# LikeLy-Journey/SegmenTron

Measured on AMD Instinct MI355X. Metric: images/sec fwd+bwd DeepLabv3+_xception65 @1025x2049, higher is better.
Workload: dtype bf16; 1 GPU; DeepLabv3+_xception65 train step (fwd + CE loss + bwd + SGD) @1025x2049, batch 2/GPU (BASELINE.json configs[2]); global_batch=2, bn=BN, parallelism=dp1, full_size=True

## Files before the change

include/segmentron_hip.h:

```cpp
#ifndef SEGMENTRON_HIP_H
#define SEGMENTRON_HIP_H
#ifdef __cplusplus
extern "C" {
#endif

const char* seg_last_error(void);
int seg_version(void);

int seg_fast_div_host(const int* s, long n, int d, int* q);
int seg_fast_div_exact(long s, long d);
int seg_fast_div_max_quot(long* out);

int seg_conv_gemm_fwd(int dtype, const void* x, long ldx, int N, int Hi, int Wi, int C,
                      const void* w, int O, int KH, int KW, int stride, int pad, int dil,
                      int pro_mode, const float* pro_scale, const float* pro_shift,
                      const float* bias, void* y, long ldy, int Ho, int Wo, int out_H, int out_W,
                      int out_s, float* stat_partial, const void* ep_x, long ldep,
                      const float* ep_c0, const float* ep_c1, int tconv, void* stream);
int seg_conv_gemm_tiles_m(int N, int Ho, int Wo);

int seg_conv_gemm_wgrad(int dtype, const void* x, long ldx, int N, int Hi, int Wi, int C,
                        const void* dy, long lddy, int Ho, int Wo, int O, int KH, int KW,
                        int stride, int pad, int dil, int pro_mode, const float* pro_scale,
                        const float* pro_shift, float* partial, int splits, void* stream);
// ... 194 lines not shown
                      const float* ta, const void* b, long ldb, const float* sb, const float* tb,
                      const void* res, long ldres, const float* w, int dil, void* ga, long ldga,
                      void* gb, long ldgb, int N, int H, int W, int n, float* pw, float* pa,
                      long pa_pitch, int pa_col, float* pb, int rows, void* stream);
int seg_fpe_bn_bwd_apply(int dtype, const void* g, long ldg, const void* x, long ldx,
                         const float* scale, const float* c0, const float* c1, void* dx, long lddx,
                         long rows, int n, void* stream);
int seg_meu_rows(int N, int h, int w, int C, int high);
int seg_meu_fwd(int dtype, const void* L, long ldl, const float* sl, const float* tl, const void* Hr,
                long ldh, const float* sh, const float* th, const float* a, const float* wsa,
                void* out, long ldo, float* sa, int N, int h, int w, int h2, int w2, int C,
                void* stream);
int seg_meu_bwd_low(int dtype, const void* g, long ldg, const void* L, long ldl, const float* sl,
                    const float* tl, const void* Hr, long ldh, const float* sh, const float* th,
                    const float* a, const float* wsa, const float* sa, void* dL, long lddl, int N,
                    int h, int w, int h2, int w2, int C, float* p_a, float* p_bn, int rows,
                    void* stream);
int seg_meu_bwd_high(int dtype, const void* g, long ldg, const float* sa, const void* Hr, long ldh,
                     const float* dpool, void* dH, long lddh, int N, int h, int w, int h2, int w2,
                     int C, float* p_bn, int rows, void* stream);

int seg_skip_pool_fwd(int dtype, const void* y, long ldy, int N, int H, int W, int C, int pro_mode,
                      const float* pro_scale, const float* pro_shift, void* skip, long ldskip,
                      void* pooled, long ldpool, void* stream);
int seg_skip_pool_bwd_rows(int dtype, int N, int H, int W, int C);
int seg_skip_pool_bwd(int dtype, const void* g_skip, long ldgs, const void* g_pool, long ldgp,
                      const void* y, long ldy, int N, int H, int W, int C, int pro_mode,
                      const float* pro_scale, const float* pro_shift, void* gx, long ldgx,
                      float* partial, int rows, void* stream);
int seg_bilinear_pad_fwd(int dtype, const void* x, long ldx, int N, int Hi, int Wi, int C,
                         int pro_mode, const float* pro_scale, const float* pro_shift, void* y,
                         long ldy, int Ho, int Wo, int Hd, int Wd, int top, int left,
                         int align_corners, void* stream);
int seg_bilinear_pad_bwd(int dtype, void* gx, long ldgx, int N, int Hi, int Wi, int C, const void* gy,
                         long ldgy, int Ho, int Wo, int Hd, int Wd, int top, int left,
                         int align_corners, void* stream);

int seg_bilinear_fwd(int dtype, const void* x, long ldx, int N, int Hi, int Wi, int C,
                     int pro_mode, const float* pro_scale, const float* pro_shift,
                     const float* chan_mul, void* y, long ldy, int Ho, int Wo, int align_corners,
                     void* stream);
int seg_bilinear_bwd(int dtype, void* gx, long ldgx, int N, int Hi, int Wi, int C, const void* gy,
                     long ldgy, int Ho, int Wo, int align_corners, void* stream);
int seg_nearest_add(int dtype, const void* x, long ldx, int mode_x, const float* sx,
                    const float* tx, const void* r, long ldr, int mode_r, const float* sr,
                    const float* tr, int shift, int post_relu, void* y, long ldy, int N, int H,
                    int W, int C, void* stream);
int seg_nearest_sum_bwd(int dtype, const void* g, long ldg, int N, int H, int W, int C, int shift,
                        void* gr, long ldgr, void* stream);
int seg_upsample_to_nchw(int dtype, const void* x, long ldx, int N, int Hi, int Wi, int C,
                         float* out, int Ho, int Wo, int align_corners, void* stream);
int seg_upsample_to_nchw_bwd(int dtype, void* gx, long ldgx, int N, int Hi, int Wi, int C,
                             const float* gy, int Ho, int Wo, int align_corners, void* stream);
int seg_nchw_to_nhwc_pad(int dtype, const float* x, int N, int Cin, int H, int W, void* y,
                         void* stream);

int seg_upsample_ce_blocks(int N, int H, int W);
int seg_upsample_ce_bwd_ws_bytes(int N, int H, int Wi, int C);
int seg_upsample_ce_fwd(int dtype, const void* lo, long ld, int N, int Hi, int Wi, int C,
                        const long* target, int H, int W, long ignore_index, int align_corners,
                        double* ws, float* loss_out, void* stream);
int seg_upsample_ce_bwd(int dtype, const void* lo, long ld, int N, int Hi, int Wi, int C,
                        const long* target, int H, int W, long ignore_index, int align_corners,
                        const float* loss_out, const float* grad_out, void* dlo, long lddlo,
                        float* ws, long ws_bytes, void* stream);

int seg_dup_ce_blocks(int dtype, long ld, int N, int h, int w, int s, int C);
int seg_dup_ce_fwd(int dtype, const void* lo, long ld, int N, int h, int w, int s, int C,
                   const long* target, long ignore_index, double* ws, float* loss_out,
                   void* stream);
int seg_dup_ce_bwd(int dtype, const void* lo, long ld, int N, int h, int w, int s, int C,
                   const long* target, long ignore_index, const float* loss_out,
                   const float* grad_out, void* dlo, long lddlo, void* stream);
int seg_dup_to_nchw(int dtype, const void* lo, long ld, int N, int h, int w, int s, int C,
                    float* out, void* stream);
int seg_dup_to_nchw_bwd(int dtype, void* gx, long ldgx, int N, int h, int w, int s, int C,
                        const float* gy, void* stream);

int seg_point_sample(int dtype_x, const void* x, long sn, long sp, long sc, int N, int H, int W,
                     int C, const float* pts, int P, int nearest, int dtype_y, void* y, long ldy,
                     int col, void* stream);
int seg_point_sample_bwd_ws(int N, int H, int W, int P);
int seg_point_sample_bwd(int dtype_g, const void* g, long ldg, int col, const float* pts, int N,
                         int P, int H, int W, int C, int dtype_x, void* dx, long lddx, int* ws,
                         void* stream);
int seg_point_uncertainty(int dtype, const void* x, long sn, long sp, long sc, int N, int H, int W,
                          int C, const float* pts, int P, float* u, void* stream);
int seg_point_topk_ws(int N, long L);
int seg_point_topk(const float* keys, int N, long L, int K, long* idx, int* ws, void* stream);
int seg_point_coords(const float* over, const long* idx, int N, int L, int K, const float* cover,
                     int P, int H, int W, float* pts, void* stream);
int seg_point_scatter(int dtype_r, const void* rend, long ldr, const long* idx, int N, int P,
                      int C, float* y, long sn, long sp, long sc, void* stream);
int seg_point_resize(int dtype, const void* x, long sn, long sp, long sc, int N, int Hi, int Wi,
                     int C, float* y, int Ho, int Wo, int align_corners, void* stream);
int seg_point_ce_blocks(long R);
int seg_point_ce_fwd(int dtype, const void* x, long ldx, long R, int C, const long* target,
                     long ignore_index, double* ws, float* loss_out, void* stream);
int seg_point_ce_bwd(int dtype, const void* x, long ldx, long R, int C, const long* target,
                     long ignore_index, const float* loss_out, const float* grad_out, void* dx,
                     long lddx, void* stream);

int seg_dwconv3x3_s2_grid_y(int C, int N, int H, int W);
int seg_dwconv3x3_s2_bwd_fused(int dtype, const void* dy, long lddy, const void* x, long ldx, int N,
                               int H, int W, int C, const float* w_c9, int pro_mode,
                               const float* pro_scale, const float* pro_shift, void* g, long ldg,
// ... 97 lines not shown
```

segmentron_amd/functional.py:

```python
import contextlib
import dataclasses
import os
import weakref

import torch
import torch.distributed as dist
import torch.nn as nn

from . import hip_ops as K
from . import parallel
from .hip_ops import PRO_AFFINE, PRO_NONE, PRO_RELU


class BNState:
    __slots__ = ("gamma", "beta", "mean", "invstd", "scale", "shift", "count", "training", "group")

    def __init__(self, gamma, beta, mean, invstd, scale, shift, count, training, group=None):
        self.gamma, self.beta = gamma, beta
        self.mean, self.invstd, self.scale, self.shift = mean, invstd, scale, shift
        self.count, self.training, self.group = count, training, group


RELU, RELU6 = 1, 5


class Act:
    __slots__ = ("t", "bn", "relu", "park")

    def __init__(self, t, bn=None, relu=False, park=None):
        self.t, self.bn, self.relu = t, bn, relu
        self.park = park

    @property
    def pro(self):
        mode = (PRO_AFFINE if self.bn is not None else PRO_NONE) | int(self.relu)
        if self.bn is None:
            return (mode, None, None)
        return (mode, self.bn.scale, self.bn.shift)

    @property
    def params(self):
        if self.bn is None:
            return None, None
        return self.bn.gamma, self.bn.beta

    def with_relu(self):
        return Act(self.t, self.bn, self.relu or True)

    @property
    def shape(self):
        return self.t.shape


_sync_group = parallel.sync_group


class GradFork:
    __slots__ = ("g", "kind", "closed", "coef")
    POST, PRE, RAW, SUM = 0, 1, 2, 3

    def __init__(self, kind=0):
        self.g, self.kind, self.closed, self.coef = None, kind, False, None

    def take(self):
        g, self.g = self.g, None
        return g

    def can_park(self, kind, g, like):
        return (self.kind == kind and self.g is None and not self.closed
                and g.dtype == like.dtype and tuple(g.shape) == tuple(like.shape))


def uses_batch_stats(bn):
    return not getattr(bn, "frozen", False) and (bn.training or bn.running_mean is None)


def finish_bn(bn, partial, count, mean_offset=None, y=None):
    use_batch = uses_batch_stats(bn)
    if not use_batch:
        scale, shift = eval_affine(bn)
        invstd = mean = None
        if torch.is_grad_enabled():
            mean = bn.running_mean
            invstd = torch.rsqrt(bn.running_var + bn.eps)
        return BNState(bn.weight, bn.bias, mean, invstd, scale, shift, count, False)
    if count <= 1 and _sync_group(bn) is None:
        raise ValueError("Expected more than 1 value per channel when training, got count=%d"
                         % count)
    group = _sync_group(bn)
    cnt = float(count)
    momentum = bn.momentum if bn.momentum is not None else 0.1
    track = bn.training and getattr(bn, "track_running_stats", False) \
        and bn.running_mean is not None
    rm, rv = (bn.running_mean, bn.running_var) if track else (None, None)
    if track:
        note_running_stats_changed()
    if group is None and y is not None and count <= K.SMALL_BN_ROWS:
        mean, invstd, scale, shift = K.bn_finalize_small(y, bn.weight, bn.bias, bn.eps, momentum,
                                                         rm, rv, mean_offset)
    elif group is None:
        mean, invstd, scale, shift = K.bn_finalize_p(partial, cnt, bn.weight, bn.bias, bn.eps,
                                                     momentum, rm, rv, mean_offset)
    else:
        C = partial.shape[-1]
        naive = parallel.is_naive_sync(bn)
        if naive:
            rm = rv = None
        box = parallel.mailbox(group)
        small = y is not None and count * dist.get_world_size(group) <= K.SMALL_BN_ROWS
        if box is not None and small:
            mean, invstd, scale, shift, cnt = K.bn_finalize_small_sync(
                box, y, bn.weight, bn.bias, bn.eps, momentum, rm, rv, mean_offset)
# ... 430 lines not shown
        else:
            dy_full = dy
        Cx = x.shape[-1]
        Ow = dy_full.shape[-1]
        dWp = K.conv_wgrad(x, dy_full, Ow, KH, KW, s.stride, s.pad, s.dil, s.pro)[:O]
        G = s.groups
        if G > 1:
            dW = block_diag_grad(dWp.view(O, Cx), G)
        elif KH == 1 and KW == 1 and Cx == Cw:
            dW = dWp.view(O, Cw, 1, 1)
        else:
            dW = dWp.view(O, KH, KW, Cx)[..., :Cw].permute(0, 3, 1, 2).contiguous()
        dbias = None
        if ctx.has_bias and s.drop_bias:
            dbias = torch.zeros(O, dtype=torch.float32, device=dy.device)
        elif ctx.has_bias:
            dbias = K.bn_bwd_reduce(dy_full, dy_full, (PRO_NONE, None, None))[:O].float()
        dx = dgamma = dbeta = None
        if ctx.needs_input_grad[0]:
            Op, dt = dy_full.shape[-1], x.dtype

            def rows(w2d):
                return w2d if Cx == Cw else torch.nn.functional.pad(w2d, (0, 0, 0, Cx - Cw))
            if G > 1:
                wt = cached_pack(weight, ("dgrad_bd", G, Op, dt), lambda: pack_conv_weight_dgrad(
                    block_diag_weight(weight, G), Op, dt))
            elif KH == 1 and KW == 1 and Op == O and Cx == Cw and weight.dtype == torch.float32:
                wt = packed_pointwise(weight, True, dt)
            else:
                wt = cached_pack(weight, ("dgrad", Op, dt, Cx),
                                 lambda: rows(pack_conv_weight_dgrad(weight, Op, dt)))
            res = None
            if s.fork is not None and s.fork.g is not None:
                res = s.fork.take()
            inplace = res is not None and getattr(s.fork, "inplace", False) \
                and tuple(res.shape) == tuple(x.shape) and _sum_n_operand_ok(res, K.vec_of(dt))
            if s.stride == 1 and res is not None and KH == 1 and KW == 1 and s.bn_in is None \
                    and not s.relu and (Cx == Cw or inplace) and Cx % K.vec_of(dt) == 0 \
                    and res.dtype == dt:
                g, _ = K.conv_gemm(dy_full, wt, Cx, 1, 1, 1, 0, 1, out=res if inplace else None,
                                   ep=(res, _const(Cx, x.device, 0.0), _const(Cx, x.device, -1.0)))
                res = None
            elif s.stride == 1:
                g, _ = K.conv_gemm(dy_full, wt, Cx, KH, KW, 1, s.dil * (KH - 1) - s.pad, s.dil)
            elif KH == 1 and KW == 1 and s.pad == 0:
                g, _ = K.conv_gemm(dy_full, wt, Cx, 1, 1, 1, 0, 1,
                                   scatter=(x.shape[1], x.shape[2], s.stride))
            else:
                wt = cached_pack(weight, ("tconv", Op, dt, Cx),
                                 lambda: rows(pack_conv_weight_tconv(weight, Op, dt)))
                g, _ = K.conv_gemm(dy_full, wt, Cx, KH, KW, s.stride, s.pad, s.dil,
                                   tconv_out_hw=(x.shape[1], x.shape[2]))
            p = s.park
            if res is None and p is not None and p.kind in (GradFork.SUM, GradFork.PRE) \
                    and p.can_park(p.kind, g, x):
                if p.kind == GradFork.PRE:
                    bn = s.bn_in
                    mode = PRO_AFFINE | int(s.relu)
                    partial = K.bn_bwd_reduce_partial(g, x, (mode, bn.scale, bn.shift))
                    dgamma, dbeta, c0, c1, _ = _bn_bwd_finish(partial, bn)
                    p.coef = (mode, c0, c1)
                p.g = g
                return None, dgamma, dbeta, dW, dbias, None
            dx, dgamma, dbeta = bn_input_backward(g, x, s.bn_in, s.relu, inplace=True)
            if res is not None:
                dx = dx + res
        elif s.fork is not None:
            s.fork.g = None
        return dx, dgamma, dbeta, dW, dbias, None


_ONES = {}


def _const(c, device, value):
    key = (c, str(device), float(value))
    if key not in _ONES:
        _ONES[key] = torch.full((c,), float(value), dtype=torch.float32, device=device)
    return _ONES[key]


def _ones(c, device):
    return _const(c, device, 1.0)


class _FoldConvFn(torch.autograd.Function):

    @staticmethod
    def forward(ctx, x, in_gamma, in_beta, weight, spec):
        O, C = weight.shape[0], weight.shape[1]
        bn = spec.bn_in
        w2d = weight.detach().view(O, C)
        wp, wpt, bp = K.fold_weights(w2d, bn.scale, bn.shift, x.dtype,
                                     want_transpose=ctx.needs_input_grad[0])
        spec.mean_offset = bp
        bias = None if spec.drop_const else bp
        y, spec.partial = K.conv_gemm(x, wp, O, 1, 1, spec.stride, 0, 1, None, bias, spec.out,
                                      spec.want_stats)
        spec.out = None
        ctx.spec = spec
        ctx.wpt = wpt
        ctx.save_for_backward(x, weight)
        return y

    @staticmethod
    def backward(ctx, dy):
        x, weight = ctx.saved_tensors
        s = ctx.spec
        bn = s.bn_in
        O, C = weight.shape[0], weight.shape[1]
        if K.nhwc(dy)[4] % K.vec_of(dy.dtype) != 0:
            dy = dy.contiguous()
        dwp = K.conv_wgrad(x, dy, O, 1, 1, s.stride, 0, 1, None, raw_partial=True)
        db = None
        if not s.drop_const:
            db = K.bn_bwd_reduce(dy, dy, (PRO_NONE, None, None))[:O].float()
        dW, dsdt = K.fold_bwd_reduce(weight.detach().view(O, C), dwp, bn.scale, bn.shift, db)
        if _bn_sums_exchanged_in_kernel(bn):
            dgamma, dbeta, c0, c1 = K.fold_bwd_finalize_sync(
                parallel.mailbox(bn.group), dsdt, bn.count, bn.mean, bn.invstd, bn.gamma, bn.scale,
                parallel.grad_scale(bn.group))
        else:
# ... 1910 lines not shown
```

segmentron_amd/hip_ops.py:

```python
import torch

from ._lib import LIB

PRO_NONE, PRO_RELU, PRO_AFFINE, PRO_AFFINE_RELU = 0, 1, 2, 3
_DT = {torch.float32: 0, torch.bfloat16: 1}


def vec_of(dtype):
    return 8 if dtype == torch.bfloat16 else 4


_raw_stream = getattr(torch._C, "_cuda_getCurrentRawStream", None)


def _stream():
    if _raw_stream is not None:
        return _raw_stream(torch.cuda.current_device())
    return torch.cuda.current_stream().cuda_stream


def _p(t):
    return 0 if t is None else t.data_ptr()


# ... 958 lines not shown
    return torch.tensor([[float(a * b) for b in ws] for a in hs], device=device)


def bilinear(x, out_hw, pro=None, chan_mul=None, align_corners=True, out=None):
    N, Hi, Wi, C, ldx = nhwc(x)
    Ho, Wo = out_hw
    mode, s, t = _pro(pro)
    if out is None:
        out = torch.empty((N, Ho, Wo, C), dtype=x.dtype, device=x.device)
    ldy = nhwc(out)[4]
    LIB.call("seg_bilinear_fwd", _DT[x.dtype], _p(x), ldx, N, Hi, Wi, C, mode, _p(s), _p(t),
             _p(chan_mul), _p(out), ldy, Ho, Wo, int(align_corners), _stream())
    return out


def bilinear_bwd(gy, in_hw, align_corners=True):
    N, Ho, Wo, C, ldgy = nhwc(gy)
    Hi, Wi = in_hw
    gx = torch.empty((N, Hi, Wi, C), dtype=gy.dtype, device=gy.device)
    LIB.call("seg_bilinear_bwd", _DT[gy.dtype], _p(gx), C, N, Hi, Wi, C, _p(gy), ldgy, Ho, Wo,
             int(align_corners), _stream())
    return gx


def upsample_to_nchw(x, C, out_hw, align_corners=True):
    N, Hi, Wi, _, ldx = nhwc(x)
    Ho, Wo = out_hw
    out = torch.empty((N, C, Ho, Wo), dtype=torch.float32, device=x.device)
    LIB.call("seg_upsample_to_nchw", _DT[x.dtype], _p(x), ldx, N, Hi, Wi, C, _p(out), Ho, Wo,
             int(align_corners), _stream())
    return out


def upsample_to_nchw_bwd(gy, in_hw, dtype, pitch, align_corners=True):
    if not gy.is_cuda or gy.dtype != torch.float32:
        raise RuntimeError("upsample_to_nchw_bwd needs a float32 HIP device tensor")
    N, C, Ho, Wo = gy.shape
    Hi, Wi = in_hw
    gy = gy.contiguous()
    gx = torch.empty((N, Hi, Wi, pitch), dtype=dtype, device=gy.device)
    LIB.call("seg_upsample_to_nchw_bwd", _DT[dtype], _p(gx), pitch, N, Hi, Wi, C, _p(gy), Ho, Wo,
             int(align_corners), _stream())
    return gx


def nchw_to_nhwc_pad(x, dtype):
    if not x.is_cuda:
        raise RuntimeError("segmentron_amd ops need HIP device tensors (no CPU fallback)")
    N, Cin, H, W = x.shape
    x = x.contiguous().float()
    y = torch.empty((N, H, W, vec_of(dtype)), dtype=dtype, device=x.device)
    LIB.call("seg_nchw_to_nhwc_pad", _DT[dtype], _p(x), N, Cin, H, W, _p(y), _stream())
    return y


def upsample_ce_fwd(lo, target, out_hw, ignore_index, align_corners=True):
    N, Hi, Wi, C, ld = nhwc(lo)
    H, W = out_hw
    if not target.is_cuda or target.dtype != torch.int64 or tuple(target.shape) != (N, H, W):
        raise RuntimeError("upsample_ce: target must be an int64 HIP tensor [N, H, W] = %s, got %s"
                           % ((N, H, W), tuple(target.shape)))
    target = target.contiguous()
    blocks = LIB.query("seg_upsample_ce_blocks", N, H, W)
    ws = torch.empty(2 * blocks, dtype=torch.float64, device=lo.device)
    out = torch.empty(2, dtype=torch.float32, device=lo.device)
    LIB.call("seg_upsample_ce_fwd", _DT[lo.dtype], _p(lo), ld, N, Hi, Wi, C, _p(target), H, W,
             int(ignore_index), int(align_corners), _p(ws), _p(out), _stream())
    return out


def upsample_ce_bwd(lo, target, out_hw, ignore_index, loss_out, grad_out, pitch,
                    align_corners=True):
    N, Hi, Wi, C, ld = nhwc(lo)
    H, W = out_hw
    grad_out = grad_out.reshape(1).to(torch.float32).contiguous()
    dlo = torch.empty((N, Hi, Wi, pitch), dtype=lo.dtype, device=lo.device)
    ws_bytes = LIB.query("seg_upsample_ce_bwd_ws_bytes", N, H, Wi, C)
    if ws_bytes < 0:
        raise RuntimeError("upsample_ce_bwd: workspace for N=%d H=%d Wi=%d C=%d exceeds 2 GiB"
                           % (N, H, Wi, C))
    ws = torch.empty((ws_bytes + 3) // 4, dtype=torch.float32, device=lo.device)
    LIB.call("seg_upsample_ce_bwd", _DT[lo.dtype], _p(lo), ld, N, Hi, Wi, C,
             _p(target.contiguous()), H, W, int(ignore_index), int(align_corners), _p(loss_out),
             _p(grad_out), _p(dlo), pitch, _p(ws), ws_bytes, _stream())
    return dlo


def _dup_geometry(lo, s, C, what):
    N, h, w, K, ld = nhwc(lo)
    if lo.dtype not in _DT:
        raise RuntimeError("%s: float32 or bfloat16 logits, got %s" % (what, lo.dtype))
    if K != s * s * C:
        raise RuntimeError("%s: %d channels are not s*s*C = %d*%d*%d" % (what, K, s, s, C))
    return N, h, w, ld


def dup_ce_fwd(lo, target, s, C, ignore_index):
    N, h, w, ld = _dup_geometry(lo, s, C, "dup_ce")
    if not target.is_cuda or target.dtype != torch.int64 \
            or tuple(target.shape) != (N, h * s, w * s):
        raise RuntimeError("dup_ce: target must be an int64 HIP tensor [N, H, W] = %s, got %s"
                           % ((N, h * s, w * s), tuple(target.shape)))
    blocks = LIB.query("seg_dup_ce_blocks", _DT[lo.dtype], ld, N, h, w, s, C)
    ws = torch.empty(2 * max(blocks, 1), dtype=torch.float64, device=lo.device)
    out = torch.empty(2, dtype=torch.float32, device=lo.device)
    LIB.call("seg_dup_ce_fwd", _DT[lo.dtype], _p(lo), ld, N, h, w, s, C, _p(target.contiguous()),
# ... 750 lines not shown
```

segmentron_amd/models/backbones/xception.py:

```python
import torch
import torch.nn as nn

from ... import functional as F
from ...config import cfg
from ...modules import SeparableConv2d
from .build import BACKBONE_REGISTRY

__all__ = ["Xception65", "XceptionBlock", "xception65"]


class XceptionBlock(nn.Module):

    def __init__(self, channel_list, stride=1, dilation=1, skip_connection_type="conv",
                 relu_first=True, low_feat=False, norm_layer=nn.BatchNorm2d):
        super().__init__()
        assert len(channel_list) == 4
        if skip_connection_type not in ("conv", "sum", "none"):
            raise ValueError("Unsupported skip connection type.")
        self.skip_connection_type = skip_connection_type
        self.relu_first = relu_first
        self.low_feat = low_feat
        c = channel_list
        if skip_connection_type == "conv":
            self.conv = nn.Conv2d(c[0], c[3], 1, stride=stride, bias=False)
# ... 23 lines not shown
        if self.low_feat:
            if self.relu_first:
                low_fork = F.low_feat_fork(sc2, self.sep_conv3.block.depthwise)
            t = F.fork(sc2.t, 2)
            sc2 = F.Act(t[0], sc2.bn, sc2.relu)
            low = F.Act(t[1], sc2.bn, sc2.relu, park=low_fork)
        residual = self.sep_conv3(sc2, fork=low_fork) if low_fork is not None \
            else self.sep_conv3(sc2)
        if self.skip_connection_type == "conv":
            shortcut = F.conv_bn(skip_in, self.conv, self.bn, park=fork)
            outputs = F.Act(F.materialize(residual, residual=shortcut))
        elif self.skip_connection_type == "sum":
            outputs = F.Act(F.materialize(residual, residual=inputs, fork=fork))
        else:
            outputs = residual
        return (outputs, low) if self.low_feat else outputs


class Xception65(nn.Module):

    def __init__(self, norm_layer=nn.BatchNorm2d):
        super().__init__()
        os_ = cfg.MODEL.OUTPUT_STRIDE
        if os_ == 32:
            b3_stride, mid_dil, exit_dil, exit_stride = 2, 1, (1, 1), 2
        elif os_ == 16:
            b3_stride, mid_dil, exit_dil, exit_stride = 2, 1, (1, 2), 1
        elif os_ == 8:
            b3_stride, mid_dil, exit_dil, exit_stride = 1, 2, (2, 4), 1
        else:
            raise NotImplementedError
        self.conv1 = nn.Conv2d(3, 32, 3, stride=2, padding=1, bias=False)
        self.bn1 = norm_layer(32)
        self.relu = nn.ReLU()
        self.conv2 = nn.Conv2d(32, 64, 3, stride=1, padding=1, bias=False)
        self.bn2 = norm_layer(64)
        self.block1 = XceptionBlock([64, 128, 128, 128], stride=2, norm_layer=norm_layer)
        self.block2 = XceptionBlock([128, 256, 256, 256], stride=2, low_feat=True,
                                    norm_layer=norm_layer)
        self.block3 = XceptionBlock([256, 728, 728, 728], stride=b3_stride, low_feat=True,
                                    norm_layer=norm_layer)
        for i in range(4, 20):
            setattr(self, "block%d" % i,
                    XceptionBlock([728] * 4, dilation=mid_dil, skip_connection_type="sum",
                                  norm_layer=norm_layer))
        self.block20 = XceptionBlock([728, 728, 1024, 1024], stride=exit_stride,
                                     dilation=exit_dil[0], norm_layer=norm_layer)
        self.block21 = XceptionBlock([1024, 1536, 1536, 2048], dilation=exit_dil[1],
                                     skip_connection_type="none", relu_first=False,
                                     norm_layer=norm_layer)

    def forward(self, x):
        from ... import compute_dtype
        a = F.Act(F.image_to_nhwc(x, compute_dtype()))
        a = F.conv_bn(a, self.conv1, self.bn1)
        a.relu = True
        a = F.conv_bn(a, self.conv2, self.bn2)
        a.relu = True
        a = self.block1(a)
        a, c1 = self.block2(a)
        a, c2 = self.block3(a)
        for i in range(4, 20):
            a = getattr(self, "block%d" % i)(a)
        c3 = a
        a = self.block20(c3)
        c4 = self.block21(a)
        return c1, c2, c3, c4


@BACKBONE_REGISTRY.register()
def xception65(norm_layer=nn.BatchNorm2d):
    return Xception65(norm_layer=norm_layer)
```

Measured before the change: 91.45 images/sec.

## Add dedicated fused stem conv kernels reading fp32 NCHW image directly

Adds a specialized HIP kernel for the 3->32 stride-2 3x3 stem convolution that reads the fp32 NCHW image directly, builds an LDS window, computes the conv with MFMA, and emits BN batch statistics. This replaces the image-to-NHWC pad pass plus a generic implicit-GEMM conv with a badly padded K dimension. A matching weight-gradient kernel takes the parked BatchNorm-backward coefficients, applying the ReLU/affine BN backward inline rather than materialising the pre-BN gradient. It adds a new GradFork kind and more complex gradient-parking logic, which could break if the stem output had other consumers.

```diff
diff --git a/include/segmentron_hip.h b/include/segmentron_hip.h
--- a/include/segmentron_hip.h
+++ b/include/segmentron_hip.h
@@ -270,6 +270,15 @@
                          float* out, int Ho, int Wo, int align_corners, void* stream);
 int seg_upsample_to_nchw_bwd(int dtype, void* gx, long ldgx, int N, int Hi, int Wi, int C,
                              const float* gy, int Ho, int Wo, int align_corners, void* stream);
+int seg_stem_conv_fwd(const float* x, int N, int H, int W, const float* w, void* y, long ldy,
+                      float* stat_partial, int stat_rows, void* stream);
+int seg_stem_conv_stat_rows(int N, int Ho, int Wo);
+int seg_stem_conv_wgrad(const float* x, int N, int H, int W, const void* g, long ldg,
+                        const void* y1, long ldy1, int mode, const float* scale,
+                        const float* shift, const float* c0, const float* c1, float* partial,
+                        int rows, void* stream);
+int seg_stem_conv_wgrad_rows(int N, int Ho, int Wo);
+int seg_stem_conv_tile(int which);
 int seg_nchw_to_nhwc_pad(int dtype, const float* x, int N, int Cin, int H, int W, void* y,
                          void* stream);
 
diff --git a/segmentron_amd/csrc/stem.hip b/segmentron_amd/csrc/stem.hip
--- /dev/null
+++ b/segmentron_amd/csrc/stem.hip
@@ -0,0 +1,416 @@
+#include "common.h"
+
+namespace seg {
+
+constexpr int ST_O = 32, ST_K = 27;
+constexpr int ST_TH = 8, ST_TW = 32, ST_THREADS = 256;
+constexpr int ST_WH = 2 * ST_TH + 1, ST_WW = 2 * ST_TW + 1;
+constexpr int ST_WP = ST_WW + 1;
+constexpr int ST_PLANE = ST_WH * ST_WP;
+constexpr int ST_WROWS = 3 * ST_WH;
+constexpr int ST_WIN_PER = (ST_WROWS + 3) / 4;
+constexpr int ST_WIN_BYTES = (3 * ST_PLANE * 2 + 15) / 16 * 16;
+constexpr int ST_OP = ST_O * 2 + 16;
+constexpr int ST_PIX_BYTES = ST_TH * ST_TW * ST_OP;
+constexpr int ST_LDS_BYTES = ST_WIN_BYTES + ST_PIX_BYTES;
+constexpr int ST_FWD_MAX_BLOCKS = 1024;
+constexpr int ST_WG_MAX_BLOCKS = 512;
+static_assert(ST_THREADS == 4 * 64 && ST_TH == 2 * 4, "a wave owns two tile rows");
+static_assert(ST_WW == 64 + 1 && ST_WROWS <= ST_THREADS, "lane = window column, + the last one");
+static_assert(4 * ST_O * 32 * 4 <= ST_PIX_BYTES, "the wave partials of the weight gradient");
+
+typedef __attribute__((address_space(3))) unsigned char st_lds_t;
+typedef short st_v4i16 __attribute__((ext_vector_type(4)));
+typedef short st_v8i16 __attribute__((ext_vector_type(8)));
+
+__host__ __device__ __forceinline__ int st_tiles(int Ho, int Wo, int* th, int* tw) {
+  *th = (Ho + ST_TH - 1) / ST_TH;
+  *tw = (Wo + ST_TW - 1) / ST_TW;
+  return *th * *tw;
+}
+
+static int st_blocks(int N, int Ho, int Wo, int cap) {
+  int th, tw;
+  const long nt = (long)N * st_tiles(Ho, Wo, &th, &tw);
+  return (int)(nt < cap ? nt : cap);
+}
+
+__device__ __forceinline__ long st_win_off(int n, int row, int h0, int wi, bool okw, int H, int W,
+                                           bool& ok) {
+  const int pl = row / ST_WH, r = row - pl * ST_WH;
+  const int hi = 2 * h0 - 1 + r;
+  ok = row < ST_WROWS && hi >= 0 && hi < H && okw;
+  return ok ? (((long)n * 3 + pl) * H + hi) * W + wi : 0;
+}
+
+__device__ __forceinline__ void st_win_load(const float* __restrict__ X, int n, int h0, int w0,
+                                            int H, int W, int tid, int wave,
+                                            float (&v)[ST_WIN_PER + 1], unsigned& okm) {
+  const int lane = tid & 63;
+  const int wi = 2 * w0 - 1 + lane, wl = 2 * w0 - 1 + (ST_WW - 1);
+  const bool okw = wi >= 0 && wi < W;
+  okm = 0;
+  bool ok;
+#pragma unroll
+  for (int q = 0; q < ST_WIN_PER; ++q) {
+    v[q] = X[st_win_off(n, wave + 4 * q, h0, wi, okw, H, W, ok)];
+    okm |= ok ? (1u << q) : 0u;
+  }
+  v[ST_WIN_PER] = X[st_win_off(n, tid, h0, wl, wl < W, H, W, ok)];
+  okm |= ok ? (1u << ST_WIN_PER) : 0u;
+}
+
+__device__ __forceinline__ void st_win_store(bf16_t* win, int tid, int wave,
+                                             const float (&v)[ST_WIN_PER + 1], unsigned okm) {
+  const int lane = tid & 63;
+#pragma unroll
+  for (int q = 0; q < ST_WIN_PER; ++q) {
+    const int row = wave + 4 * q;
+    const bf16_t b = ((okm >> q) & 1u) ? f32_to_bf16(v[q]) : (bf16_t)0;
+    if (row < ST_WROWS) win[row * ST_WP + lane] = b;
+  }
+  const bf16_t b = ((okm >> ST_WIN_PER) & 1u) ? f32_to_bf16(v[ST_WIN_PER]) : (bf16_t)0;
+  if (tid < ST_WROWS) win[tid * ST_WP + (ST_WW - 1)] = b;
+}
+
+__device__ __forceinline__ int st_koff(int k) {
+  const int c = k / 9, t = k - c * 9;
+  const int kh = t / 3, kw = t - kh * 3;
+  return (c * ST_WH + kh) * ST_WP + kw;
+}
+
+__device__ __forceinline__ bf16x8 st_gather8(const bf16_t* p, const int (&o)[8], unsigned zero) {
+  uint32_t u[4];
+#pragma unroll
+  for (int i = 0; i < 4; ++i) {
+    uint32_t lo = p[o[2 * i]], hi = p[o[2 * i + 1]];
+    lo = ((zero >> (2 * i)) & 1u) ? 0u : lo;
+    hi = ((zero >> (2 * i + 1)) & 1u) ? 0u : hi;
+    u[i] = lo | (hi << 16);
+  }
+  return __builtin_bit_cast(bf16x8, make_uint4(u[0], u[1], u[2], u[3]));
+}
+
+__device__ __forceinline__ void st_tile_range(int ntiles, int& t0, int& t1) {
+  const int nblk = gridDim.x;
+  const int L = xcd_remap(blockIdx.x, nblk);
+  t0 = (int)((long)L * ntiles / nblk);
+  t1 = (int)((long)(L + 1) * ntiles / nblk);
+}
+
+__device__ __forceinline__ void st_tile_origin(int t, int tiles_h, int tiles_w, int& n, int& h0,
+                                               int& w0) {
+  const int tw = t % tiles_w, tq = t / tiles_w;
+  const int th = tq % tiles_h;
+  n = tq / tiles_h;
+  h0 = th * ST_TH;
+  w0 = tw * ST_TW;
+}
+
+template <bool STATS>
+__global__ __launch_bounds__(ST_THREADS, 4) void stem_conv_fwd_kernel(
+    const float* __restrict__ X, const float* __restrict__ Wt, bf16_t* __restrict__ Y, long ldy,
+    float* __restrict__ partial, int H, int W, int Ho, int Wo, int tiles_h, int tiles_w,
+    int ntiles) {
+  __shared__ __attribute__((aligned(16))) unsigned char st_smem[ST_LDS_BYTES];
+  const int tid = threadIdx.x, lane = tid & 63;
+  const int wave = __builtin_amdgcn_readfirstlane(tid >> 6);
+  const int r32 = lane & 31, h = lane >> 5;
+  bf16_t* win = reinterpret_cast<bf16_t*>(st_smem);
+  unsigned char* patch = st_smem + ST_WIN_BYTES + wave * (2 * ST_TW * ST_OP);
+
+  bf16x8 wf[2];
+  int koff[2][8];
+  unsigned kzero[2];
+#pragma unroll
+  for (int ks = 0; ks < 2; ++ks) {
+    float w[8];
+    kzero[ks] = 0;
+#pragma unroll
+    for (int j = 0; j < 8; ++j) {
+      const int k = ks * 16 + h * 8 + j;
+      const bool real = k < ST_K;
+      const float v = Wt[r32 * ST_K + (real ? k : 0)];
+      w[j] = real ? v : 0.f;
+      koff[ks][j] = real ? st_koff(k) : 0;
+      kzero[ks] |= real ? 0u : (1u << j);
+    }
+    wf[ks] = __builtin_bit_cast(bf16x8, Vec<bf16_t>::pack(w));
+  }
+  float s1[16], s2[16];
+#pragma unroll
+  for (int e = 0; e < 16; ++e) s1[e] = s2[e] = 0.f;
+
+  int t0, t1, n, h0, w0;
+  st_tile_range(ntiles, t0, t1);
+  for (int t = t0; t < t1; ++t) {
+    st_tile_origin(t, tiles_h, tiles_w, n, h0, w0);
+    {
+      float v[ST_WIN_PER + 1];
+      unsigned okm;
+      st_win_load(X, n, h0, w0, H, W, tid, wave, v, okm);
+      st_win_store(win, tid, wave, v, okm);
+    }
+    __syncthreads();
+
+#pragma unroll 1
+    for (int rr = 0; rr < 2; ++rr) {
+      const int r = wave * 2 + rr;
+      const bf16_t* base = win + (2 * r) * ST_WP + 2 * r32;
+      f32x16 acc;
+#pragma unroll
+      for (int e = 0; e < 16; ++e) acc[e] = 0.f;
+#pragma unroll
+      for (int ks = 0; ks < 2; ++ks) {
+        const bf16x8 b = st_gather8(base, koff[ks], kzero[ks]);
+        acc = __builtin_amdgcn_mfma_f32_32x32x16_bf16(wf[ks], b, acc, 0, 0, 0);
+      }
+      if (STATS) {
+        const bool valid = h0 + r < Ho && w0 + r32 < Wo;
+#pragma unroll
+        for (int e = 0; e < 16; ++e) {
+          const float v = valid ? acc[e] : 0.f;
+          s1[e] += v;
+          s2[e] = fmaf(v, v, s2[e]);
+        }
+      }
+#pragma unroll
+      for (int g = 0; g < 4; ++g) {
+        const uint2 pk = make_uint2(pack_bf16x2(acc[g * 4 + 0], acc[g * 4 + 1]),
+                                    pack_bf16x2(acc[g * 4 + 2], acc[g * 4 + 3]));
+        *reinterpret_cast<uint2*>(patch + (rr * ST_TW + r32) * ST_OP + (g * 8 + h * 4) * 2) = pk;
+      }
+    }
+    __syncthreads();
+#pragma unroll
+    for (int it = 0; it < 4; ++it) {
+      const int rr = it >> 1, px = (it & 1) * 16 + (lane >> 2), v = lane & 3;
+      const int ho = h0 + wave * 2 + rr, wo = w0 + px;
+      const uint4 val = *reinterpret_cast<const uint4*>(patch + (rr * ST_TW + px) * ST_OP + v * 16);
+      if (ho < Ho && wo < Wo) stg16(Y + (((long)n * Ho + ho) * Wo + wo) * ldy + v * 8, val);
+    }
+  }
+
+  if (STATS) {
+#pragma unroll
+    for (int e = 0; e < 16; ++e) {
+#pragma unroll
+      for (int m = 1; m < 32; m <<= 1) {
+        s1[e] += __shfl_xor(s1[e], m, 64);
+        s2[e] += __shfl_xor(s2[e], m, 64);
+      }
+    }
+    __syncthreads();
+    float* red = reinterpret_cast<float*>(st_smem);
+    if (r32 == 0) {
+#pragma unroll
+      for (int e = 0; e < 16; ++e) {
+        const int c = (e >> 2) * 8 + h * 4 + (e & 3);
+        red[(wave * 2 + 0) * ST_O + c] = s1[e];
+        red[(wave * 2 + 1) * ST_O + c] = s2[e];
+      }
+    }
+    __syncthreads();
+    if (tid < 2 * ST_O) {
+      float s = 0.f;
+      for (int w = 0; w < 4; ++w) s += red[w * 2 * ST_O + tid];
+      partial[(long)blockIdx.x * 2 * ST_O + tid] = s;
+    }
+  }
+}
+
+__device__ __forceinline__ bf16x8 st_tr_frag(const st_lds_t* p, int second_off) {
+  typedef __attribute__((address_space(3))) st_v4i16 lds_v4;
+  const st_v4i16 lo = __builtin_amdgcn_ds_read_tr16_b64_v4i16((lds_v4*)p);
+  const st_v4i16 hi = __builtin_amdgcn_ds_read_tr16_b64_v4i16((lds_v4*)(p + second_off));
+  const st_v8i16 v = {lo.x, lo.y, lo.z, lo.w, hi.x, hi.y, hi.z, hi.w};
+  return __builtin_bit_cast(bf16x8, v);
+}
+
+__global__ __launch_bounds__(ST_THREADS, 2) void stem_conv_wgrad_kernel(
+    const float* __restrict__ X, const bf16_t* __restrict__ G, long ldg,
+    const bf16_t* __restrict__ Y1, long ldy1, int mode, const float* __restrict__ scale,
+    const float* __restrict__ shift, const float* __restrict__ c0p, const float* __restrict__ c1p,
+    float* __restrict__ partial, int H, int W, int Ho, int Wo, int tiles_h, int tiles_w,
+    int ntiles) {
+  __shared__ __attribute__((aligned(16))) unsigned char st_smem[ST_LDS_BYTES];
+  const int tid = threadIdx.x, lane = tid & 63;
+  const int wave = __builtin_amdgcn_readfirstlane(tid >> 6);
+  const int r32 = lane & 31, h = lane >> 5;
+  bf16_t* win = reinterpret_cast<bf16_t*>(st_smem);
+  unsigned char* ds = st_smem + ST_WIN_BYTES;
+
+  const int cvec = tid & 3;
+  float sc[8], sh[8], k0[8], k1[8];
+#pragma unroll
+  for (int i = 0; i < 8; ++i) { sc[i] = 1.f; sh[i] = 0.f; k0[i] = k1[i] = 0.f; }
+  if (mode & PRO_AFFINE) {
+    load_params<8>(scale, cvec * 8, sc);
+    load_params<8>(shift, cvec * 8, sh);
+  }
+  if (c0p) {
+    load_params<8>(c0p, cvec * 8, k0);
+    load_params<8>(c1p, cvec * 8, k1);
+  }
+  const bool kreal = r32 < ST_K;
+  const int kbase = (kreal ? st_koff(r32) : 0) + 2 * (h * 8);
+  const unsigned kzero = kreal ? 0u : 0xFFu;
+  int poff[8];
+#pragma unroll
+  for (int j = 0; j < 8; ++j) poff[j] = 2 * j;
+  const int tg = lane >> 4, ti = lane & 15;
+  const st_lds_t* a_base =
+      (const st_lds_t*)ds + (8 * (tg >> 1) + (ti >> 2)) * ST_OP + ((tg & 1) * 16 + (ti & 3) * 4) * 2;
+
+  f32x16 acc;
+#pragma unroll
+  for (int e = 0; e < 16; ++e) acc[e] = 0.f;
+
+  float v[ST_WIN_PER + 1];
+  unsigned okm, okd;
+  uint4 rg[4], ry[4];
+  auto load_tile = [&](int t) {
+    int n, h0, w0;
+    st_tile_origin(t, tiles_h, tiles_w, n, h0, w0);
+    st_win_load(X, n, h0, w0, H, W, tid, wave, v, okm);
+    okd = 0;
+#pragma unroll
+    for (int q = 0; q < 4; ++q) {
+      const int pix = (tid >> 2) + 64 * q;
+      const int ho = h0 + (pix >> 5), wo = w0 + (pix & 31);
+      const bool ok = ho < Ho && wo < Wo;
+      const long p = ok ? ((long)n * Ho + ho) * Wo + wo : 0;
+      rg[q] = ldg16(G + p * ldg + cvec * 8);
+      ry[q] = ldg16(Y1 + p * ldy1 + cvec * 8);
+      okd |= ok ? (1u << q) : 0u;
+    }
+  };
+  int t0, t1;
+  st_tile_range(ntiles, t0, t1);
+  for (int t = t0; t < t1; ++t) {
+    load_tile(t);
+    {
+      st_win_store(win, tid, wave, v, okm);
+#pragma unroll
+      for (int q = 0; q < 4; ++q) {
+        const int pix = (tid >> 2) + 64 * q;
+        float g[8], x[8];
+        Vec<bf16_t>::unpack(rg[q], g);
+        Vec<bf16_t>::unpack(ry[q], x);
+        if (mode & PRO_RELU) {
+#pragma unroll
+          for (int k = 0; k < 8; ++k) {
+            const float y = (mode & PRO_AFFINE) ? fmaf(x[k], sc[k], sh[k]) : x[k];
+            const bool on = y > 0.f && (!(mode & PRO_CLAMP6) || y < 6.f);
+            g[k] = on ? g[k] : 0.f;
+          }
+        }
+        if (mode & PRO_AFFINE) {
+#pragma unroll
+          for (int k = 0; k < 8; ++k) g[k] = g[k] * sc[k] - k0[k] - k1[k] * x[k];
+        }
+        *reinterpret_cast<uint4*>(ds + pix * ST_OP + cvec * 16) =
+            mask_u4(Vec<bf16_t>::pack(g), (okd >> q) & 1u);
+      }
+    }
+    __syncthreads();
+#pragma unroll
+    for (int rr = 0; rr < 2; ++rr) {
+      const int r = wave * 2 + rr;
+#pragma unroll
+      for (int hf = 0; hf < 2; ++hf) {
+        const bf16x8 fa = st_tr_frag(a_base + (r * ST_TW + hf * 16) * ST_OP, 4 * ST_OP);
+        const bf16x8 fb = st_gather8(win + kbase + (2 * r) * ST_WP + 2 * (hf * 16), poff, kzero);
+        acc = __builtin_amdgcn_mfma_f32_32x32x16_bf16(fa, fb, acc, 0, 0, 0);
+      }
+    }
+    __syncthreads();
+  }
+
+  float* red = reinterpret_cast<float*>(ds);
+#pragma unroll
+  for (int e = 0; e < 16; ++e) {
+    const int o = (e & 3) + 8 * (e >> 2) + 4 * h;
+    red[(wave * ST_O + o) * 32 + r32] = acc[e];
+  }
+  __syncthreads();
+  float* P = partial + (long)blockIdx.x * (ST_O * ST_K);
+  for (int idx = tid; idx < ST_O * ST_K; idx += ST_THREADS) {
+    const int o = idx / ST_K, k = idx - o * ST_K;
+    float s = 0.f;
+    for (int w = 0; w < 4; ++w) s += red[(w * ST_O + o) * 32 + k];
+    P[idx] = s;
+  }
+}
+
+}
+
+static int stem_geometry(const char* what, int N, int H, int W, int* Ho, int* Wo) {
+  SEG_REQUIRE(N >= 1 && H >= 1 && W >= 1, "%s: empty image %d x %d x %d", what, N, H, W);
+  *Ho = (H - 1) / 2 + 1;
+  *Wo = (W - 1) / 2 + 1;
+  SEG_REQUIRE((long)N * *Ho * *Wo < (1L << 31) / seg::ST_O, "%s: %d x %d x %d pixels overflow", what,
+              N, *Ho, *Wo);
+  return 0;
+}
+
+extern "C" int seg_stem_conv_stat_rows(int N, int Ho, int Wo) {
+  return seg::st_blocks(N, Ho, Wo, seg::ST_FWD_MAX_BLOCKS);
+}
+
+extern "C" int seg_stem_conv_wgrad_rows(int N, int Ho, int Wo) {
+  return seg::st_blocks(N, Ho, Wo, seg::ST_WG_MAX_BLOCKS);
+}
+
+extern "C" int seg_stem_conv_fwd(const float* x, int N, int H, int W, const float* w, void* y,
+                                 long ldy, float* stat_partial, int stat_rows, void* stream) {
+  using namespace seg;
+  int Ho, Wo, th, tw;
+  if (stem_geometry("stem_conv_fwd", N, H, W, &Ho, &Wo)) return 1;
+  SEG_REQUIRE(x != nullptr && w != nullptr && y != nullptr, "stem_conv_fwd: null x / w / y");
+  SEG_REQUIRE(ldy >= ST_O && ldy % 8 == 0, "stem_conv_fwd: output pitch %ld", ldy);
+  const int ntiles = N * st_tiles(Ho, Wo, &th, &tw);
+  const int blocks = st_blocks(N, Ho, Wo, ST_FWD_MAX_BLOCKS);
+  SEG_REQUIRE(stat_partial == nullptr || stat_rows == blocks,
+              "stem_conv_fwd: %d statistics rows, the launch writes %d (seg_stem_conv_stat_rows)",
+              stat_rows, blocks);
+  hipStream_t s = static_cast<hipStream_t>(stream);
+  if (stat_partial)
+    hipLaunchKernelGGL((stem_conv_fwd_kernel<true>), dim3(blocks), dim3(ST_THREADS), 0, s, x, w,
+                       static_cast<bf16_t*>(y), ldy, stat_partial, H, W, Ho, Wo, th, tw, ntiles);
+  else
+    hipLaunchKernelGGL((stem_conv_fwd_kernel<false>), dim3(blocks), dim3(ST_THREADS), 0, s, x, w,
+                       static_cast<bf16_t*>(y), ldy, stat_partial, H, W, Ho, Wo, th, tw, ntiles);
+  return check_launch("stem_conv_fwd");
+}
+
+extern "C" int seg_stem_conv_wgrad(const float* x, int N, int H, int W, const void* g, long ldg,
+                                   const void* y1, long ldy1, int mode, const float* scale,
+                                   const float* shift, const float* c0, const float* c1,
+                                   float* partial, int rows, void* stream) {
+  using namespace seg;
+  int Ho, Wo, th, tw;
+  if (stem_geometry("stem_conv_wgrad", N, H, W, &Ho, &Wo)) return 1;
+  SEG_REQUIRE(x != nullptr && g != nullptr && y1 != nullptr && partial != nullptr,
+              "stem_conv_wgrad: null x / g / y1 / partial");
+  SEG_REQUIRE(ldg >= ST_O && ldg % 8 == 0 && ldy1 >= ST_O && ldy1 % 8 == 0,
+              "stem_conv_wgrad: pitches %ld / %ld", ldg, ldy1);
+  SEG_REQUIRE(mode >= 0 && mode < 8 && (!(mode & PRO_CLAMP6) || (mode & PRO_RELU)),
+              "stem_conv_wgrad: bad prologue mode %d", mode);
+  SEG_REQUIRE(!(mode & PRO_AFFINE) || (scale != nullptr && shift != nullptr),
+              "stem_conv_wgrad: affine mode without scale / shift");
+  SEG_REQUIRE((c0 == nullptr) == (c1 == nullptr) && (c0 == nullptr || (mode & PRO_AFFINE)),
+              "stem_conv_wgrad: c0 and c1 go together, with an affine mode");
+  const int ntiles = N * st_tiles(Ho, Wo, &th, &tw);
+  const int blocks = st_blocks(N, Ho, Wo, ST_WG_MAX_BLOCKS);
+  SEG_REQUIRE(rows == blocks,
+              "stem_conv_wgrad: %d partial rows, the launch writes %d (seg_stem_conv_wgrad_rows)",
+              rows, blocks);
+  hipLaunchKernelGGL(stem_conv_wgrad_kernel, dim3(blocks), dim3(ST_THREADS), 0,
+                     static_cast<hipStream_t>(stream), x, static_cast<const bf16_t*>(g), ldg,
+                     static_cast<const bf16_t*>(y1), ldy1, mode, scale, shift, c0, c1, partial, H, W,
+                     Ho, Wo, th, tw, ntiles);
+  return check_launch("stem_conv_wgrad");
+}
+
+extern "C" int seg_stem_conv_tile(int which) { return which == 0 ? seg::ST_TH : seg::ST_TW; }
diff --git a/segmentron_amd/functional.py b/segmentron_amd/functional.py
--- a/segmentron_amd/functional.py
+++ b/segmentron_amd/functional.py
@@ -57,7 +57,7 @@
 
 class GradFork:
     __slots__ = ("g", "kind", "closed", "coef")
-    POST, PRE, RAW, SUM = 0, 1, 2, 3
+    POST, PRE, RAW, SUM, STEM = 0, 1, 2, 3, 4
 
     def __init__(self, kind=0):
         self.g, self.kind, self.closed, self.coef = None, kind, False, None
@@ -594,6 +594,21 @@
                 g, _ = K.conv_gemm(dy_full, wt, Cx, KH, KW, s.stride, s.pad, s.dil,
                                    tconv_out_hw=(x.shape[1], x.shape[2]))
             p = s.park
+            if p is not None and p.kind == GradFork.STEM and p.g is not None:
+                raise RuntimeError("the BatchNorm-backward coefficients parked for the image "
+                                   "stem's weight gradient were not taken")
+            if res is None and p is not None and p.kind == GradFork.STEM \
+                    and s.bn_in is not None and p.can_park(GradFork.STEM, g, x) \
+                    and not _bn_is_few_sample(s.bn_in, g.shape[0] * g.shape[1] * g.shape[2]):
+                bn = s.bn_in
+                mode = PRO_AFFINE | int(s.relu)
+                partial = K.bn_bwd_reduce_partial(g, x, (mode, bn.scale, bn.shift))
+                dgamma, dbeta, c0, c1, _ = _bn_bwd_finish(partial, bn)
+                if not bn.training:
+                    c0 = c1 = None
+                p.coef = (mode, bn.scale, bn.shift, c0, c1, x)
+                p.g = g
+                return g, dgamma, dbeta, dW, dbias, None
             if res is None and p is not None and p.kind in (GradFork.SUM, GradFork.PRE) \
                     and p.can_park(p.kind, g, x):
                 if p.kind == GradFork.PRE:
@@ -610,6 +625,71 @@
         elif s.fork is not None:
             s.fork.g = None
         return dx, dgamma, dbeta, dW, dbias, None
+
+
+class StemSpec:
+    def __init__(self, want_stats, fork):
+        self.want_stats, self.fork, self.partial = want_stats, fork, None
+
+
+class _StemFn(torch.autograd.Function):
+
+    @staticmethod
+    def forward(ctx, image, weight, spec):
+        y, spec.partial = K.stem_conv_fwd(image, weight.detach().contiguous(), spec.want_stats)
+        ctx.spec = spec
+        ctx.save_for_backward(image)
+        return y
+
+    @staticmethod
+    def backward(ctx, dy):
+        image, = ctx.saved_tensors
+        f = ctx.spec.fork
+        if K.nhwc(dy)[4] % K.vec_of(dy.dtype) != 0:
+            dy = dy.contiguous()
+        if f is not None and f.g is not None:
+            g, coef, f.coef = f.take(), f.coef, None
+            mode, scale, shift, c0, c1, y1 = coef
+            if g.data_ptr() != dy.data_ptr() or tuple(g.shape) != tuple(dy.shape):
+                raise RuntimeError("the image stem's output has a second consumer: the gradient "
+                                   "parked with its BatchNorm-backward coefficients is not the "
+                                   "one autograd delivered")
+            dW = K.stem_conv_wgrad(image, g, y1, (mode, scale, shift), c0, c1)
+        else:
+            dW = K.stem_conv_wgrad(image, dy)
+        return None, dW, None
+
+
+def stem_conv_routed(image, conv, bn, dtype):
+    if not (torch.is_tensor(image) and image.is_cuda and image.dim() == 4 and image.shape[1] == 3
+            and image.dtype == torch.float32 and not image.requires_grad
+            and dtype == torch.bfloat16):
+        return False
+    if not (isinstance(conv, nn.Conv2d) and conv.in_channels == 3 and conv.out_channels == K.STEM_O
+            and tuple(conv.kernel_size) == (3, 3) and tuple(conv.stride) == (2, 2)
+            and tuple(conv.padding) == (1, 1) and tuple(conv.dilation) == (1, 1)
+            and conv.groups == 1 and conv.bias is None and conv.padding_mode == "zeros"
+            and conv.weight.dtype == torch.float32):
+        return False
+    if bn is None or is_group_norm(bn):
+        return False
+    N, _, H, W = image.shape
+    return N * ((H - 1) // 2 + 1) * ((W - 1) // 2 + 1) > K.SMALL_BN_ROWS
+
+
+def stem_conv_bn(image, conv, bn, dtype=None):
+    if dtype is None:
+        from . import compute_dtype
+        dtype = compute_dtype()
+    if not stem_conv_routed(image, conv, bn, dtype):
+        return conv_bn(Act(image_to_nhwc(image, dtype)), conv, bn)
+    fork = None
+    if torch.is_grad_enabled() and conv.weight.requires_grad:
+        fork = GradFork(GradFork.STEM)
+    spec = StemSpec(uses_batch_stats(bn), fork)
+    y = _StemFn.apply(image.contiguous(), conv.weight, spec)
+    N, Ho, Wo, _ = y.shape
+    return Act(y, finish_bn(bn, spec.partial, N * Ho * Wo, y=y), park=fork)
 
 
 _ONES = {}
diff --git a/segmentron_amd/hip_ops.py b/segmentron_amd/hip_ops.py
--- a/segmentron_amd/hip_ops.py
+++ b/segmentron_amd/hip_ops.py
@@ -1034,6 +1034,53 @@
     y = torch.empty((N, H, W, vec_of(dtype)), dtype=dtype, device=x.device)
     LIB.call("seg_nchw_to_nhwc_pad", _DT[dtype], _p(x), N, Cin, H, W, _p(y), _stream())
     return y
+
+
+STEM_O = 32
+
+
+def _stem_image(x):
+    if not x.is_cuda:
+        raise RuntimeError("segmentron_amd ops need HIP device tensors (no CPU fallback)")
+    if x.dim() != 4 or x.shape[1] != 3 or x.dtype != torch.float32 or not x.is_contiguous():
+        raise RuntimeError("stem_conv: expected a contiguous float32 NCHW image with 3 channels, "
+                           "got %s %s" % (tuple(x.shape), x.dtype))
+    N, _, H, W = x.shape
+    return N, H, W, (H - 1) // 2 + 1, (W - 1) // 2 + 1
+
+
+def stem_conv_fwd(x, w, want_stats=False):
+    N, H, W, Ho, Wo = _stem_image(x)
+    assert tuple(w.shape) == (STEM_O, 3, 3, 3) and w.dtype == torch.float32 and w.is_contiguous()
+    y = torch.empty((N, Ho, Wo, STEM_O), dtype=torch.bfloat16, device=x.device)
+    partial, rows = None, 0
+    if want_stats:
+        rows = LIB.query("seg_stem_conv_stat_rows", N, Ho, Wo)
+        partial = torch.empty((rows, 2, STEM_O), dtype=torch.float32, device=x.device)
+    LIB.call("seg_stem_conv_fwd", _p(x), N, H, W, _p(w), _p(y), STEM_O, _p(partial), rows,
+             _stream())
+    return y, partial
+
+
+def stem_conv_wgrad(x, g, y1=None, pro=None, c0=None, c1=None):
+    N, H, W, Ho, Wo = _stem_image(x)
+    Ng, Hg, Wg, Cg, ldg = nhwc(g)
+    assert (Ng, Hg, Wg, Cg) == (N, Ho, Wo, STEM_O) and g.dtype == torch.bfloat16
+    mode, ps, pt = _pro(pro)
+    if y1 is None:
+        assert mode == PRO_NONE and c0 is None and c1 is None
+        y1 = g
+    assert tuple(y1.shape) == tuple(g.shape) and y1.dtype == g.dtype
+    rows = LIB.query("seg_stem_conv_wgrad_rows", N, Ho, Wo)
+    partial = torch.empty((rows, STEM_O * 27), dtype=torch.float32, device=x.device)
+    LIB.call("seg_stem_conv_wgrad", _p(x), N, H, W, _p(g), ldg, _p(y1), nhwc(y1)[4], int(mode),
+             _p(ps), _p(pt), _p(c0), _p(c1), _p(partial), rows, _stream())
+    dW = partial[0] if rows == 1 else colsum(partial, f64=False)
+    return dW.view(STEM_O, 3, 3, 3)
+
+
+def stem_conv_tile():
+    return LIB.query("seg_stem_conv_tile", 0), LIB.query("seg_stem_conv_tile", 1)
 
 
 def upsample_ce_fwd(lo, target, out_hw, ignore_index, align_corners=True):
diff --git a/segmentron_amd/models/backbones/xception.py b/segmentron_amd/models/backbones/xception.py
--- a/segmentron_amd/models/backbones/xception.py
+++ b/segmentron_amd/models/backbones/xception.py
@@ -99,8 +99,7 @@
 
     def forward(self, x):
         from ... import compute_dtype
-        a = F.Act(F.image_to_nhwc(x, compute_dtype()))
-        a = F.conv_bn(a, self.conv1, self.bn1)
+        a = F.stem_conv_bn(x, self.conv1, self.bn1, compute_dtype())
         a.relu = True
         a = F.conv_bn(a, self.conv2, self.bn2)
         a.relu = True
```

Measured after the change: 92.13 images/sec (median of 6 runs). About the same (+0.7%).
